# MARSLab-UMN/vi_depth_completion

Hardware: AMD Instinct MI355X
Metric: frames/sec (higher is better)
Workload: dtype f32

## Files before the change

vi_depth_completion_amd/csrc/wfused.hip:

```cpp
#include "common.h"
#include <cstdlib>

#pragma clang fp contract(off)

namespace {

typedef float f32x4 __attribute__((ext_vector_type(4)));

constexpr int TB = 16, NBW = 32, KC = 16, NPOS = 36;
constexpr int NPW = 8, NTW = 8, NTHREADS = 64 * (NPW + NTW);
constexpr int VBUF = NPOS * TB * KC;
constexpr int XSLOT = 37;
constexpr int XBUF = TB * XSLOT * KC;
constexpr int NDMA = TB * XSLOT / 16;
constexpr int MLD = 36;
constexpr size_t LDS_BYTES = (size_t)(2 * VBUF + 2 * XBUF) * sizeof(float);
static_assert(TB * XSLOT % 16 == 0, "whole DMA instructions");
static_assert((size_t)NPOS * TB * MLD * sizeof(float) <= LDS_BYTES, "the epilogue's product rows reuse the buffers");
static_assert(LDS_BYTES <= 160 * 1024, "one workgroup per CU");

struct FArgs {
    const float* x; const float* u; float* y; const float* s1; const float* b1; const float* s2; const float* b2;
    int H, W, Cin, ldx, Cout, ldy, th, tw, T, flags, nbn, gn;
    long long x_gs, w_gs, y_gs, p_gs;
    unsigned x_bytes;
};

typedef __attribute__((address_space(3))) void lds_void_t;

template <typename V> __device__ __forceinline__ void bt6_lo(const V (&d)[6], V (&t)[3]) {
    const V p = d[4] - 4.f * d[2], q = d[3] - 4.f * d[1];
    t[0] = (4.f * d[0] - 5.f * d[2]) + d[4];
    t[1] = p + q;
    t[2] = p - q;
}
template <typename V> __device__ __forceinline__ void bt6_hi(const V (&d)[6], V (&t)[3]) {
    const V r = d[4] - d[2], s = 2.f * (d[3] - d[1]);
    t[0] = r + s;
    t[1] = r - s;
    t[2] = (4.f * d[1] - 5.f * d[3]) + d[5];
}
template <typename V> __device__ __forceinline__ void bt6(const V (&d)[6], V (&t)[6]) {
    V lo[3], hi[3];
    bt6_lo(d, lo);
    bt6_hi(d, hi);
#pragma unroll
    for (int i = 0; i < 3; ++i) { t[i] = lo[i]; t[3 + i] = hi[i]; }
}
__device__ __forceinline__ void at6(const float (&m)[6], float (&o)[4]) {
    const float s12 = m[1] + m[2], d12 = m[1] - m[2], s34 = m[3] + m[4], d34 = m[3] - m[4];
    o[0] = (m[0] + s12) + s34;
    o[1] = d12 + 2.f * d34;
    o[2] = s12 + 4.f * s34;
    o[3] = (d12 + 8.f * d34) + m[5];
}

template <int N_> __device__ __forceinline__ void wait_lgkmcnt() { asm volatile("s_waitcnt lgkmcnt(%0)" ::"n"(N_) : "memory"); }
__device__ __forceinline__ f32x4 lds_read_b128(unsigned addr) {
    f32x4 v;
    asm volatile("ds_read_b128 %0, %1" : "=v"(v) : "v"(addr));
    return v;
}
template <int OFF> __device__ __forceinline__ float lds_read_b32(unsigned addr) {
    float v;
    asm volatile("ds_read_b32 %0, %1 offset:%2" : "=v"(v) : "v"(addr), "n"(OFF));
    return v;
}
template <int OFF> __device__ __forceinline__ void lds_write_b32(unsigned addr, float v) { asm volatile("ds_write_b32 %0, %1 offset:%2" ::"v"(addr), "v"(v), "n"(OFF) : "memory"); }

template <int PW, int NB, int DBG>
__device__ __forceinline__ void product_wave(const FArgs& a, float* smem, unsigned lds0, int lane, int pos0, int g, int nb, int NK) {
    const int n = lane & 15, kq = lane >> 4;
    const int n32 = a.Cout / 32, pair = NB == 2 ? nb : nb >> 1, half = NB == 2 ? 0 : nb & 1;
    const float* ub = a.u + (size_t)g * a.w_gs + ((size_t)pos0 * n32 + pair) * ((size_t)NK * 512) + half * 256 + lane * 4;
    const size_t pos_stride = (size_t)n32 * NK * 512;
    auto load_b = [&](int p, int kc, f32x4 (&dst)[NB]) {
        const float* s = ub + (size_t)p * pos_stride + (size_t)kc * 512;
        dst[0] = *reinterpret_cast<const f32x4*>(s);
        if constexpr (NB == 2) dst[1] = *reinterpret_cast<const f32x4*>(s + 256);
    };
    f32x4 acc[PW][NB];
#pragma unroll
    for (int p = 0; p < PW; ++p)
#pragma unroll
        for (int j = 0; j < NB; ++j) acc[p][j] = f32x4{0.f, 0.f, 0.f, 0.f};
    f32x4 bq[PW][NB];
#pragma unroll
    for (int p = 0; p < PW; ++p) load_b(p, 0, bq[p]);
    const unsigned a_off = (unsigned)((n * KC + ((kq ^ ((n >> 2) & 3)) * 4)) * 4);
    const unsigned a_wave = lds0 + (unsigned)(pos0 * TB * KC * 4);

    __builtin_amdgcn_s_barrier();
    __builtin_amdgcn_s_barrier();
    __builtin_amdgcn_s_barrier();
    for (int kc = 0; kc < NK; ++kc) {
        const unsigned vb = a_wave + (unsigned)((kc & 1) * VBUF * 4);
        const int kn = kc + 1 < NK ? kc + 1 : kc;
        f32x4 fa[2];
        fa[0] = lds_read_b128(vb + a_off);
#pragma unroll
        for (int p = 0; p < PW; ++p) {
            const int cur = p & 1, nxt = cur ^ 1;
            if (p + 1 < PW) {
                fa[nxt] = lds_read_b128(vb + (unsigned)((p + 1) * TB * KC * 4) + a_off);
                wait_lgkmcnt<1>();
            } else {
                wait_lgkmcnt<0>();
            }
            __builtin_amdgcn_sched_barrier(0);
#pragma unroll
            for (int ks = 0; ks < 4; ++ks)
#pragma unroll
                for (int j = 0; j < NB; ++j)
                    if constexpr (!(DBG & 1)) acc[p][j] = __builtin_amdgcn_mfma_f32_16x16x4f32(fa[cur][ks], bq[p][j][ks], acc[p][j], 0, 0, 0);
                    else if (ks == 0) acc[p][j][0] += fa[cur][0] + fa[cur][3] + bq[p][j][0] + bq[p][j][3];
            if constexpr (!(DBG & 2)) load_b(p, kn, bq[p]);
            __builtin_amdgcn_sched_barrier(0);
        }
        __builtin_amdgcn_s_barrier();
    }
    asm volatile("s_waitcnt vmcnt(0)" ::: "memory");
    float* mx = smem;
#pragma unroll
    for (int p = 0; p < PW; ++p)
#pragma unroll
        for (int j = 0; j < NB; ++j)
#pragma unroll
            for (int i = 0; i < 4; ++i) mx[((pos0 + p) * TB + 4 * kq + i) * MLD + j * 16 + n] = acc[p][j][i];
}

template <int NB, int DBG>
__global__ void __launch_bounds__(NTHREADS)
wino4_fused_kernel(const FArgs a) {
    extern __shared__ __attribute__((aligned(16))) float smem[];
    const int tid = threadIdx.x;
    const int L = blockIdx.x;
    const int tb = L / a.gn, r_ = L - tb * a.gn, g = r_ / a.nbn, nb = r_ - g * a.nbn;
    const int NK = a.Cin / KC;
    const unsigned lds0 = (unsigned)(size_t)((__attribute__((address_space(3))) float*)smem);

    if (tid < 64 * NPW) {
        const int w = __builtin_amdgcn_readfirstlane(tid >> 6);
        if (w < 4) product_wave<5, NB, DBG>(a, smem, lds0, tid & 63, 5 * w, g, nb, NK);
        else product_wave<4, NB, DBG>(a, smem, lds0, tid & 63, 20 + 4 * (w - 4), g, nb, NK);
    } else {
        const int tt = tid - 64 * NPW, lane = tid & 63;
        const int w8 = __builtin_amdgcn_readfirstlane(tt >> 6), grp = w8 >> 2;
        const int u_ = tt & 255, m = u_ >> 4, c = u_ & 15;
        const int tpf = a.th * a.tw;
        constexpr unsigned OOB = 0x80000000u;
        unsigned voff[5];
#pragma unroll
        for (int i = 0; i < 5; ++i) {
            const int j = w8 + 8 * i;
            const int slot = 16 * j + (lane >> 2), quad = lane & 3;
            const int ts = slot / XSLOT, px = slot - ts * XSLOT;
            const int t = tb * TB + ts;
            bool ok = j < NDMA && px < 36 && t < a.T;
            const int tc = ok ? t : 0;
            const int b = tc / tpf, rem = tc - b * tpf, ty = rem / a.tw, tx = rem - ty * a.tw;
            const int r = px / 6, s = px - r * 6;
            const int iy = ty * 4 - 1 + r, ix = tx * 4 - 1 + s;
            ok = ok && (unsigned)iy < (unsigned)a.H && (unsigned)ix < (unsigned)a.W;
            voff[i] = ok ? (unsigned)(((size_t)((b * a.H + iy) * a.W + ix) * a.ldx + (size_t)g * a.x_gs + quad * 4) * 4) : OOB;
        }
        const __amdgpu_buffer_rsrc_t x_rsrc = __builtin_amdgcn_make_buffer_rsrc(const_cast<float*>(a.x), 0, (int)a.x_bytes, 0x00020000);
        auto dma = [&](int cc) {
            float* dst = smem + 2 * VBUF + (cc & 1) * XBUF;
            const int soff = cc * KC * 4;
#pragma unroll
            for (int i = 0; i < 5; ++i)
                if (w8 + 8 * i < NDMA) __builtin_amdgcn_raw_ptr_buffer_load_lds(x_rsrc, (lds_void_t*)(dst + (w8 + 8 * i) * 256), 16, (int)voff[i], soff, 0, 0);
        };
        float out[36];
        const unsigned x_thr = lds0 + (unsigned)((2 * VBUF + (m * XSLOT) * KC + c) * 4);
        const unsigned v_thr = lds0 + (unsigned)((m * KC + (((c >> 2) ^ ((m >> 2) & 3)) * 4) + (c & 3)) * 4);
        auto phase_a = [&](int cc) {
            const unsigned xa = x_thr + (unsigned)((cc & 1) * XBUF * 4);
            float D[36];
#define VIDC_RD(i) D[i] = lds_read_b32<(i) * KC * 4>(xa);
            VIDC_RD(0) VIDC_RD(1) VIDC_RD(2) VIDC_RD(3) VIDC_RD(4) VIDC_RD(5) VIDC_RD(6) VIDC_RD(7) VIDC_RD(8) VIDC_RD(9) VIDC_RD(10) VIDC_RD(11)
            VIDC_RD(12) VIDC_RD(13) VIDC_RD(14) VIDC_RD(15) VIDC_RD(16) VIDC_RD(17) VIDC_RD(18) VIDC_RD(19) VIDC_RD(20) VIDC_RD(21) VIDC_RD(22) VIDC_RD(23)
            VIDC_RD(24) VIDC_RD(25) VIDC_RD(26) VIDC_RD(27) VIDC_RD(28) VIDC_RD(29) VIDC_RD(30) VIDC_RD(31) VIDC_RD(32) VIDC_RD(33) VIDC_RD(34) VIDC_RD(35)
#undef VIDC_RD
            asm volatile("s_waitcnt lgkmcnt(0)" : "+v"(D[0]), "+v"(D[1]), "+v"(D[2]), "+v"(D[3]), "+v"(D[4]), "+v"(D[5]), "+v"(D[6]), "+v"(D[7]), "+v"(D[8]), "+v"(D[9]), "+v"(D[10]), "+v"(D[11]), "+v"(D[12]), "+v"(D[13]), "+v"(D[14]), "+v"(D[15]), "+v"(D[16]), "+v"(D[17]) :: "memory");
            asm volatile("" : "+v"(D[18]), "+v"(D[19]), "+v"(D[20]), "+v"(D[21]), "+v"(D[22]), "+v"(D[23]), "+v"(D[24]), "+v"(D[25]), "+v"(D[26]), "+v"(D[27]), "+v"(D[28]), "+v"(D[29]), "+v"(D[30]), "+v"(D[31]), "+v"(D[32]), "+v"(D[33]), "+v"(D[34]), "+v"(D[35]) :: "memory");
            float tcol[6][6];
#pragma unroll
            for (int s = 0; s < 6; ++s) {
                float col[6], o6[6];
#pragma unroll
                for (int r = 0; r < 6; ++r) col[r] = D[r * 6 + s];
                bt6(col, o6);
#pragma unroll
                for (int r = 0; r < 6; ++r) tcol[r][s] = o6[r];
            }
#pragma unroll
            for (int r = 0; r < 6; ++r) {
                float o6[6];
                bt6(tcol[r], o6);
#pragma unroll
                for (int s = 0; s < 6; ++s) out[r * 6 + s] = o6[s];
            }
        };
        auto phase_b = [&](int cc) {
            const unsigned va = v_thr + (unsigned)((cc & 1) * VBUF * 4);
#define VIDC_WR(i) lds_write_b32<(i) * TB * KC * 4>(va, out[i]);
            VIDC_WR(0) VIDC_WR(1) VIDC_WR(2) VIDC_WR(3) VIDC_WR(4) VIDC_WR(5) VIDC_WR(6) VIDC_WR(7) VIDC_WR(8) VIDC_WR(9) VIDC_WR(10) VIDC_WR(11)
            VIDC_WR(12) VIDC_WR(13) VIDC_WR(14) VIDC_WR(15) VIDC_WR(16) VIDC_WR(17) VIDC_WR(18) VIDC_WR(19) VIDC_WR(20) VIDC_WR(21) VIDC_WR(22) VIDC_WR(23)
            VIDC_WR(24) VIDC_WR(25) VIDC_WR(26) VIDC_WR(27) VIDC_WR(28) VIDC_WR(29) VIDC_WR(30) VIDC_WR(31) VIDC_WR(32) VIDC_WR(33) VIDC_WR(34) VIDC_WR(35)
#undef VIDC_WR
        };
        auto fence_barrier = [&]() {
            if constexpr (DBG & 16) asm volatile("s_waitcnt lgkmcnt(0)" ::: "memory");
            else asm volatile("s_waitcnt vmcnt(0) lgkmcnt(0)" ::: "memory");
            __builtin_amdgcn_s_barrier();
        };
        dma(0);
        if (NK > 1) dma(1);
        fence_barrier();
        if (grp == 0) phase_a(0);
        else if (NK > 1) phase_a(1);
        fence_barrier();
        if (NK > 2) dma(2);
        if (grp == 0) phase_b(0);
        fence_barrier();
        for (int it = 0; it < NK; ++it) {
            if (!(DBG & 4)) {
                if (it + 3 < NK) dma(it + 3);
                if ((it & 1) == grp) {
                    if (it + 2 < NK) phase_a(it + 2);
                } else {
                    if (it + 1 < NK) phase_b(it + 1);
                }
            }
            fence_barrier();
        }
    }
    __syncthreads();
    if (tid < TB * 16 * NB) {
        const int m = tid / (16 * NB), c = tid - m * (16 * NB);
        const int t = tb * TB + m;
        if (t >= a.T || (DBG & 8)) return;
        const int tpf = a.th * a.tw;
        const int b = t / tpf, rem = t - b * tpf, ty = rem / a.tw, tx = rem - ty * a.tw;
        const float* mx = smem + m * MLD + c;
        float tc[4][6];
#pragma unroll
        for (int s = 0; s < 6; ++s) {
            float col[6], o4[4];
#pragma unroll
            for (int r = 0; r < 6; ++r) col[r] = mx[(r * 6 + s) * TB * MLD];
            at6(col, o4);
#pragma unroll
            for (int r = 0; r < 4; ++r) tc[r][s] = o4[r];
        }
        const int ch = nb * 16 * NB + c;
        const float s1 = a.s1[(size_t)g * a.p_gs + ch], b1 = a.b1[(size_t)g * a.p_gs + ch];
        const bool aff2 = a.flags & VIDC_AFFINE2;
        const float s2 = aff2 ? a.s2[(size_t)g * a.p_gs + ch] : 0.f, b2 = aff2 ? a.b2[(size_t)g * a.p_gs + ch] : 0.f;
        const float lo1 = (a.flags & VIDC_RELU1) ? 0.f : -INFINITY, lo2 = (a.flags & VIDC_RELU2) ? 0.f : -INFINITY;
        float* yb = a.y + (size_t)g * a.y_gs + ch;
#pragma unroll
        for (int r = 0; r < 4; ++r) {
            float o4[4];
            at6(tc[r], o4);
            const int oy = ty * 4 + r;
            if (oy >= a.H) continue;
#pragma unroll
            for (int s = 0; s < 4; ++s) {
                const int ox = tx * 4 + s;
                if (ox >= a.W) continue;
                float o = fmaxf(o4[s] * s1 + b1, lo1);
                if (aff2) o = fmaxf(o * s2 + b2, lo2);
                yb[((size_t)(b * a.H + oy) * a.W + ox) * a.ldy] = o;
            }
        }
    }
}

__global__ void __launch_bounds__(256)
wino4_pack_kernel(const float* __restrict__ u, float* __restrict__ o, int Cout, int Cin, long long total4) {
    const long long i = (long long)blockIdx.x * blockDim.x + threadIdx.x;
    if (i >= total4) return;
    const int NK = Cin / KC, nbn = Cout / NBW;
    const int lane = (int)(i & 63), nblk = (int)((i >> 6) & 1);
    long long r = i >> 7;
    const int kc = (int)(r % NK); r /= NK;
    const int nb = (int)(r % nbn);
    const int pos = (int)(r / nbn);
    const int n = lane & 15, kq = lane >> 4;
    const float4 v = *reinterpret_cast<const float4*>(u + ((size_t)pos * Cout + nb * NBW + nblk * 16 + n) * Cin + kc * KC + kq * 4);
    *reinterpret_cast<float4*>(o + i * 4) = v;
}

template <int NB, int DBG>
int launch_nb(const FArgs& a, long long wgs, hipStream_t st) {
    static bool attr_set[64] = {};
    int dev = 0;
    VIDC_HIP(hipGetDevice(&dev));
    if (dev < 0 || dev >= 64 || !attr_set[dev]) {
        VIDC_HIP(hipFuncSetAttribute(reinterpret_cast<const void*>(&wino4_fused_kernel<NB, DBG>), hipFuncAttributeMaxDynamicSharedMemorySize, (int)LDS_BYTES));
        if (dev >= 0 && dev < 64) attr_set[dev] = true;
    }
    hipLaunchKernelGGL((wino4_fused_kernel<NB, DBG>), dim3((unsigned)wgs), dim3(NTHREADS), LDS_BYTES, st, a);
    VIDC_CHECK_LAUNCH("wino4_fused_kernel");
    return VIDC_OK;
}

template <int DBG>
int launch_dbg(const FArgs& a, long long wgs, hipStream_t st) { return a.nbn * 32 == a.Cout ? launch_nb<2, DBG>(a, wgs, st) : launch_nb<1, DBG>(a, wgs, st); }

}

namespace vidc {

int launch_wino4_fused(const vidc_conv_desc& d, hipStream_t st) {
    VIDC_REQUIRE(d.precision == VIDC_PREC_FP32, VIDC_ERR_SHAPE, "conv (fused Winograd): fp32 arithmetic only");
    VIDC_REQUIRE(d.KH == 3 && d.KW == 3 && d.stride == 1 && d.pad == 1 && d.dilation <= 1, VIDC_ERR_SHAPE, "conv (fused Winograd): 3x3 / stride 1 / pad 1 / dense only");
    VIDC_REQUIRE(d.Cin % KC == 0 && d.Cout % NBW == 0 && d.ldx % 4 == 0, VIDC_ERR_SHAPE, "conv (fused Winograd): Cin %% 16 == 0, Cout %% 32 == 0, ldx %% 4 == 0");
    VIDC_REQUIRE(!(d.flags & ~(VIDC_RELU1 | VIDC_AFFINE2 | VIDC_RELU2)), VIDC_ERR_SHAPE, "conv (fused Winograd): flags 0x%x not supported (affine / ReLU / second affine / ReLU only)", d.flags);
    VIDC_REQUIRE(d.w_gs == (long long)NPOS * d.Cout * d.Cin || d.groups == 1, VIDC_ERR_SHAPE, "conv (fused Winograd): w = U of vidc_winograd_weight_pack_fused, w_gs = 36 * Cout * Cin");
    VIDC_REQUIRE((reinterpret_cast<uintptr_t>(d.x) & 15) == 0 && (reinterpret_cast<uintptr_t>(d.w) & 15) == 0 && d.x_gs % 4 == 0, VIDC_ERR_SHAPE, "conv (fused Winograd): x and U 16-byte aligned");
    FArgs a;
    a.x = d.x; a.u = d.w; a.y = d.y; a.s1 = d.scale1; a.b1 = d.shift1; a.s2 = d.scale2; a.b2 = d.shift2;
    a.H = d.H; a.W = d.W; a.Cin = d.Cin; a.ldx = d.ldx; a.Cout = d.Cout; a.ldy = d.ldy;
    a.th = (d.H + 3) / 4; a.tw = (d.W + 3) / 4;
    a.T = d.B * a.th * a.tw;
    static const int force_nb = [] { const char* e = getenv("VIDC_WFUSED_NB"); return e ? atoi(e) : 0; }();
    const long long wgs32 = (long long)((d.B * a.th * a.tw + TB - 1) / TB) * d.groups * (d.Cout / NBW);
    const int nbk = force_nb == 1 || force_nb == 2 ? force_nb : (wgs32 * 2 <= 256 ? 1 : 2);
    a.flags = d.flags; a.nbn = d.Cout / (16 * nbk); a.gn = d.groups * a.nbn;
    a.x_gs = d.x_gs; a.w_gs = d.w_gs; a.y_gs = d.y_gs; a.p_gs = d.p_gs;
    VIDC_REQUIRE((long long)d.B * d.H * d.W * d.ldx * 4 < (1ll << 30), VIDC_ERR_SHAPE, "conv (fused Winograd): the input must stay below 1 GiB");
    a.x_bytes = (unsigned)((long long)d.B * d.H * d.W * d.ldx * 4);
    const long long wgs = (long long)((a.T + TB - 1) / TB) * a.gn;
    VIDC_REQUIRE(wgs < (1ll << 31), VIDC_ERR_SHAPE, "conv (fused Winograd): grid too large");
#ifdef VIDC_WFUSED_ATTRIB
    static const int dbg = [] { const char* e = getenv("VIDC_WFUSED_DBG"); return e ? atoi(e) : 0; }();
    switch (dbg) {
        case 1: return launch_dbg<1>(a, wgs, st);
        case 2: return launch_dbg<2>(a, wgs, st);
        case 4: return launch_dbg<4>(a, wgs, st);
        case 8: return launch_dbg<8>(a, wgs, st);
        case 3: return launch_dbg<3>(a, wgs, st);
        case 6: return launch_dbg<6>(a, wgs, st);
        case 7: return launch_dbg<7>(a, wgs, st);
        case 15: return launch_dbg<15>(a, wgs, st);
        case 16: return launch_dbg<16>(a, wgs, st);
        default: break;
    }
#endif
    return launch_dbg<0>(a, wgs, st);
}

}

extern "C" int vidc_winograd_weight_pack_fused(const float* u, float* u_packed, int Cout, int Cin, vidc_stream_t stream) {
    VIDC_REQUIRE(u && u_packed && u != u_packed, VIDC_ERR_NULL, "vidc_winograd_weight_pack_fused: null pointer (or in place)");
    VIDC_REQUIRE(Cout > 0 && Cin > 0 && Cout % NBW == 0 && Cin % KC == 0, VIDC_ERR_SHAPE, "vidc_winograd_weight_pack_fused: Cout must be a multiple of 32, Cin of 16");
    const long long total4 = (long long)NPOS * Cout * Cin / 4;
    hipLaunchKernelGGL(wino4_pack_kernel, dim3((unsigned)((total4 + 255) / 256)), dim3(256), 0, vidc::as_stream(stream), u, u_packed, Cout, Cin, total4);
    VIDC_CHECK_LAUNCH("wino4_pack_kernel");
    return VIDC_OK;
}
```

Baseline: 632.0.

## Make fused Winograd conv persistent for Cin=64 with cross-item prefetch

For Cin==64 layers the fused Winograd kernel now launches a grid sized to the CU count, rounded to a multiple of groups*nbn, and loops over tile items. Each workgroup prefetches the next item's first input chunks and weight slices while the current item's K loop finishes, so the pipeline does not drain and refill between tiles. This aims to cut workgroup launch and prologue cost. The epilogue is moved into a shared fold_store, and the product rows are stored in a compact XOR-swizzled layout that fits in the V buffers. In exchange there are extra block-wide syncs per item and possible load imbalance on the last round of items.

Result: faster. 639.5, median of 6 (+1.2%).

```diff
diff --git a/vi_depth_completion_amd/csrc/wfused.hip b/vi_depth_completion_amd/csrc/wfused.hip
--- a/vi_depth_completion_amd/csrc/wfused.hip
+++ b/vi_depth_completion_amd/csrc/wfused.hip
@@ -18,10 +18,12 @@
 static_assert(TB * XSLOT % 16 == 0, "whole DMA instructions");
 static_assert((size_t)NPOS * TB * MLD * sizeof(float) <= LDS_BYTES, "the epilogue's product rows reuse the buffers");
 static_assert(LDS_BYTES <= 160 * 1024, "one workgroup per CU");
+static_assert(NPOS * TB * 32 <= 2 * VBUF, "a persistent workgroup's product rows fit in the two V buffers");
 
 struct FArgs {
     const float* x; const float* u; float* y; const float* s1; const float* b1; const float* s2; const float* b2;
     int H, W, Cin, ldx, Cout, ldy, th, tw, T, flags, nbn, gn;
+    int items;
     long long x_gs, w_gs, y_gs, p_gs;
     unsigned x_bytes;
 };
@@ -68,9 +70,17 @@
 }
 template <int OFF> __device__ __forceinline__ void lds_write_b32(unsigned addr, float v) { asm volatile("ds_write_b32 %0, %1 offset:%2" ::"v"(addr), "v"(v), "n"(OFF) : "memory"); }
 
-template <int PW, int NB, int DBG>
-__device__ __forceinline__ void product_wave(const FArgs& a, float* smem, unsigned lds0, int lane, int pos0, int g, int nb, int NK) {
+template <bool PERSIST> __device__ __forceinline__ int prow(int pos, int m, int col) {
+    if constexpr (PERSIST) return (pos * TB + m) * 32 + (col ^ (((m >> 2) & 1) << 4));
+    else return (pos * TB + m) * MLD + col;
+}
+
+template <int NB, int DBG, bool PERSIST> __device__ void fold_store(const FArgs& a, const float* smem, int tid, int tb, int g, int nb);
+template <int PW, int NB, int DBG, bool PERSIST>
+__device__ __forceinline__ void product_wave(const FArgs& a, float* smem, unsigned lds0, int tid, int pos0, int NK) {
+    const int lane = tid & 63;
     const int n = lane & 15, kq = lane >> 4;
+    const int item0 = blockIdx.x, r0 = item0 % a.gn, g = r0 / a.nbn, nb = r0 - g * a.nbn;
     const int n32 = a.Cout / 32, pair = NB == 2 ? nb : nb >> 1, half = NB == 2 ? 0 : nb & 1;
     const float* ub = a.u + (size_t)g * a.w_gs + ((size_t)pos0 * n32 + pair) * ((size_t)NK * 512) + half * 256 + lane * 4;
     const size_t pos_stride = (size_t)n32 * NK * 512;
@@ -79,77 +89,123 @@
         dst[0] = *reinterpret_cast<const f32x4*>(s);
         if constexpr (NB == 2) dst[1] = *reinterpret_cast<const f32x4*>(s + 256);
     };
-    f32x4 acc[PW][NB];
-#pragma unroll
-    for (int p = 0; p < PW; ++p)
-#pragma unroll
-        for (int j = 0; j < NB; ++j) acc[p][j] = f32x4{0.f, 0.f, 0.f, 0.f};
     f32x4 bq[PW][NB];
 #pragma unroll
     for (int p = 0; p < PW; ++p) load_b(p, 0, bq[p]);
     const unsigned a_off = (unsigned)((n * KC + ((kq ^ ((n >> 2) & 3)) * 4)) * 4);
     const unsigned a_wave = lds0 + (unsigned)(pos0 * TB * KC * 4);
 
-    __builtin_amdgcn_s_barrier();
-    __builtin_amdgcn_s_barrier();
-    __builtin_amdgcn_s_barrier();
-    for (int kc = 0; kc < NK; ++kc) {
-        const unsigned vb = a_wave + (unsigned)((kc & 1) * VBUF * 4);
-        const int kn = kc + 1 < NK ? kc + 1 : kc;
-        f32x4 fa[2];
-        fa[0] = lds_read_b128(vb + a_off);
-#pragma unroll
-        for (int p = 0; p < PW; ++p) {
-            const int cur = p & 1, nxt = cur ^ 1;
-            if (p + 1 < PW) {
-                fa[nxt] = lds_read_b128(vb + (unsigned)((p + 1) * TB * KC * 4) + a_off);
-                wait_lgkmcnt<1>();
-            } else {
-                wait_lgkmcnt<0>();
+    for (int item = item0; item < a.items; item += gridDim.x) {
+        const bool more = PERSIST && item + (int)gridDim.x < a.items;
+        f32x4 acc[PW][NB];
+#pragma unroll
+        for (int p = 0; p < PW; ++p)
+#pragma unroll
+            for (int j = 0; j < NB; ++j) acc[p][j] = f32x4{0.f, 0.f, 0.f, 0.f};
+        __builtin_amdgcn_s_barrier();
+        __builtin_amdgcn_s_barrier();
+        __builtin_amdgcn_s_barrier();
+        for (int kc = 0; kc < NK; ++kc) {
+            const unsigned vb = a_wave + (unsigned)((kc & 1) * VBUF * 4);
+            const int kn = kc + 1 < NK ? kc + 1 : (more ? 0 : kc);
+            f32x4 fa[2];
+            fa[0] = lds_read_b128(vb + a_off);
+#pragma unroll
+            for (int p = 0; p < PW; ++p) {
+                const int cur = p & 1, nxt = cur ^ 1;
+                if (p + 1 < PW) {
+                    fa[nxt] = lds_read_b128(vb + (unsigned)((p + 1) * TB * KC * 4) + a_off);
+                    wait_lgkmcnt<1>();
+                } else {
+                    wait_lgkmcnt<0>();
+                }
+                __builtin_amdgcn_sched_barrier(0);
+#pragma unroll
+                for (int ks = 0; ks < 4; ++ks)
+#pragma unroll
+                    for (int j = 0; j < NB; ++j)
+                        if constexpr (!(DBG & 1)) acc[p][j] = __builtin_amdgcn_mfma_f32_16x16x4f32(fa[cur][ks], bq[p][j][ks], acc[p][j], 0, 0, 0);
+                        else if (ks == 0) acc[p][j][0] += fa[cur][0] + fa[cur][3] + bq[p][j][0] + bq[p][j][3];
+                if constexpr (!(DBG & 2)) load_b(p, kn, bq[p]);
+                __builtin_amdgcn_sched_barrier(0);
             }
-            __builtin_amdgcn_sched_barrier(0);
-#pragma unroll
-            for (int ks = 0; ks < 4; ++ks)
-#pragma unroll
-                for (int j = 0; j < NB; ++j)
-                    if constexpr (!(DBG & 1)) acc[p][j] = __builtin_amdgcn_mfma_f32_16x16x4f32(fa[cur][ks], bq[p][j][ks], acc[p][j], 0, 0, 0);
-                    else if (ks == 0) acc[p][j][0] += fa[cur][0] + fa[cur][3] + bq[p][j][0] + bq[p][j][3];
-            if constexpr (!(DBG & 2)) load_b(p, kn, bq[p]);
-            __builtin_amdgcn_sched_barrier(0);
-        }
-        __builtin_amdgcn_s_barrier();
-    }
-    asm volatile("s_waitcnt vmcnt(0)" ::: "memory");
-    float* mx = smem;
-#pragma unroll
-    for (int p = 0; p < PW; ++p)
-#pragma unroll
-        for (int j = 0; j < NB; ++j)
-#pragma unroll
-            for (int i = 0; i < 4; ++i) mx[((pos0 + p) * TB + 4 * kq + i) * MLD + j * 16 + n] = acc[p][j][i];
-}
-
-template <int NB, int DBG>
+            __builtin_amdgcn_s_barrier();
+        }
+        asm volatile("s_waitcnt vmcnt(0)" ::: "memory");
+#pragma unroll
+        for (int p = 0; p < PW; ++p)
+#pragma unroll
+            for (int j = 0; j < NB; ++j)
+#pragma unroll
+                for (int i = 0; i < 4; ++i) smem[prow<PERSIST>(pos0 + p, 4 * kq + i, j * 16 + n)] = acc[p][j][i];
+        __syncthreads();
+        fold_store<NB, DBG, PERSIST>(a, smem, tid, item / a.gn, g, nb);
+        if constexpr (PERSIST) __syncthreads();
+    }
+}
+
+template <int NB, int DBG, bool PERSIST>
+__device__ void fold_store(const FArgs& a, const float* smem, int tid, int tb, int g, int nb) {
+    if (tid >= TB * 16 * NB) return;
+    const int m = tid / (16 * NB), c = tid - m * (16 * NB);
+    const int t = tb * TB + m;
+    if (t >= a.T || (DBG & 8)) return;
+    const int tpf = a.th * a.tw;
+    const int b = t / tpf, rem = t - b * tpf, ty = rem / a.tw, tx = rem - ty * a.tw;
+    float tc[4][6];
+#pragma unroll
+    for (int s = 0; s < 6; ++s) {
+        float col[6], o4[4];
+#pragma unroll
+        for (int r = 0; r < 6; ++r) col[r] = smem[prow<PERSIST>(r * 6 + s, m, c)];
+        at6(col, o4);
+#pragma unroll
+        for (int r = 0; r < 4; ++r) tc[r][s] = o4[r];
+    }
+    const int ch = nb * 16 * NB + c;
+    const float s1 = a.s1[(size_t)g * a.p_gs + ch], b1 = a.b1[(size_t)g * a.p_gs + ch];
+    const bool aff2 = a.flags & VIDC_AFFINE2;
+    const float s2 = aff2 ? a.s2[(size_t)g * a.p_gs + ch] : 0.f, b2 = aff2 ? a.b2[(size_t)g * a.p_gs + ch] : 0.f;
+    const float lo1 = (a.flags & VIDC_RELU1) ? 0.f : -INFINITY, lo2 = (a.flags & VIDC_RELU2) ? 0.f : -INFINITY;
+    float* yb = a.y + (size_t)g * a.y_gs + ch;
+#pragma unroll
+    for (int r = 0; r < 4; ++r) {
+        float o4[4];
+        at6(tc[r], o4);
+        const int oy = ty * 4 + r;
+        if (oy >= a.H) continue;
+#pragma unroll
+        for (int s = 0; s < 4; ++s) {
+            const int ox = tx * 4 + s;
+            if (ox >= a.W) continue;
+            float o = fmaxf(o4[s] * s1 + b1, lo1);
+            if (aff2) o = fmaxf(o * s2 + b2, lo2);
+            yb[((size_t)(b * a.H + oy) * a.W + ox) * a.ldy] = o;
+        }
+    }
+}
+
+template <int NB, int DBG, bool PERSIST>
 __global__ void __launch_bounds__(NTHREADS)
 wino4_fused_kernel(const FArgs a) {
     extern __shared__ __attribute__((aligned(16))) float smem[];
     const int tid = threadIdx.x;
-    const int L = blockIdx.x;
-    const int tb = L / a.gn, r_ = L - tb * a.gn, g = r_ / a.nbn, nb = r_ - g * a.nbn;
     const int NK = a.Cin / KC;
     const unsigned lds0 = (unsigned)(size_t)((__attribute__((address_space(3))) float*)smem);
 
     if (tid < 64 * NPW) {
         const int w = __builtin_amdgcn_readfirstlane(tid >> 6);
-        if (w < 4) product_wave<5, NB, DBG>(a, smem, lds0, tid & 63, 5 * w, g, nb, NK);
-        else product_wave<4, NB, DBG>(a, smem, lds0, tid & 63, 20 + 4 * (w - 4), g, nb, NK);
-    } else {
-        const int tt = tid - 64 * NPW, lane = tid & 63;
-        const int w8 = __builtin_amdgcn_readfirstlane(tt >> 6), grp = w8 >> 2;
-        const int u_ = tt & 255, m = u_ >> 4, c = u_ & 15;
-        const int tpf = a.th * a.tw;
-        constexpr unsigned OOB = 0x80000000u;
-        unsigned voff[5];
+        if (w < 4) product_wave<5, NB, DBG, PERSIST>(a, smem, lds0, tid, 5 * w, NK);
+        else product_wave<4, NB, DBG, PERSIST>(a, smem, lds0, tid, 20 + 4 * (w - 4), NK);
+        return;
+    }
+    const int tt = tid - 64 * NPW, lane = tid & 63;
+    const int w8 = __builtin_amdgcn_readfirstlane(tt >> 6), grp = w8 >> 2;
+    const int u_ = tt & 255, m = u_ >> 4, c = u_ & 15;
+    const int tpf = a.th * a.tw;
+    const int g = (blockIdx.x % a.gn) / a.nbn;
+    constexpr unsigned OOB = 0x80000000u;
+    auto offsets = [&](int tb, unsigned (&voff)[5]) {
 #pragma unroll
         for (int i = 0; i < 5; ++i) {
             const int j = w8 + 8 * i;
@@ -164,70 +220,83 @@
             ok = ok && (unsigned)iy < (unsigned)a.H && (unsigned)ix < (unsigned)a.W;
             voff[i] = ok ? (unsigned)(((size_t)((b * a.H + iy) * a.W + ix) * a.ldx + (size_t)g * a.x_gs + quad * 4) * 4) : OOB;
         }
-        const __amdgpu_buffer_rsrc_t x_rsrc = __builtin_amdgcn_make_buffer_rsrc(const_cast<float*>(a.x), 0, (int)a.x_bytes, 0x00020000);
-        auto dma = [&](int cc) {
-            float* dst = smem + 2 * VBUF + (cc & 1) * XBUF;
-            const int soff = cc * KC * 4;
-#pragma unroll
-            for (int i = 0; i < 5; ++i)
-                if (w8 + 8 * i < NDMA) __builtin_amdgcn_raw_ptr_buffer_load_lds(x_rsrc, (lds_void_t*)(dst + (w8 + 8 * i) * 256), 16, (int)voff[i], soff, 0, 0);
-        };
-        float out[36];
-        const unsigned x_thr = lds0 + (unsigned)((2 * VBUF + (m * XSLOT) * KC + c) * 4);
-        const unsigned v_thr = lds0 + (unsigned)((m * KC + (((c >> 2) ^ ((m >> 2) & 3)) * 4) + (c & 3)) * 4);
-        auto phase_a = [&](int cc) {
-            const unsigned xa = x_thr + (unsigned)((cc & 1) * XBUF * 4);
-            float D[36];
+    };
+    const __amdgpu_buffer_rsrc_t x_rsrc = __builtin_amdgcn_make_buffer_rsrc(const_cast<float*>(a.x), 0, (int)a.x_bytes, 0x00020000);
+    auto dma = [&](const unsigned (&voff)[5], int cc) {
+        float* dst = smem + 2 * VBUF + (cc & 1) * XBUF;
+        const int soff = cc * KC * 4;
+#pragma unroll
+        for (int i = 0; i < 5; ++i)
+            if (w8 + 8 * i < NDMA) __builtin_amdgcn_raw_ptr_buffer_load_lds(x_rsrc, (lds_void_t*)(dst + (w8 + 8 * i) * 256), 16, (int)voff[i], soff, 0, 0);
+    };
+    float out[36];
+    const unsigned x_thr = lds0 + (unsigned)((2 * VBUF + (m * XSLOT) * KC + c) * 4);
+    const unsigned v_thr = lds0 + (unsigned)((m * KC + (((c >> 2) ^ ((m >> 2) & 3)) * 4) + (c & 3)) * 4);
+    auto phase_a = [&](int cc) {
+        const unsigned xa = x_thr + (unsigned)((cc & 1) * XBUF * 4);
+        float D[36];
 #define VIDC_RD(i) D[i] = lds_read_b32<(i) * KC * 4>(xa);
-            VIDC_RD(0) VIDC_RD(1) VIDC_RD(2) VIDC_RD(3) VIDC_RD(4) VIDC_RD(5) VIDC_RD(6) VIDC_RD(7) VIDC_RD(8) VIDC_RD(9) VIDC_RD(10) VIDC_RD(11)
-            VIDC_RD(12) VIDC_RD(13) VIDC_RD(14) VIDC_RD(15) VIDC_RD(16) VIDC_RD(17) VIDC_RD(18) VIDC_RD(19) VIDC_RD(20) VIDC_RD(21) VIDC_RD(22) VIDC_RD(23)
-            VIDC_RD(24) VIDC_RD(25) VIDC_RD(26) VIDC_RD(27) VIDC_RD(28) VIDC_RD(29) VIDC_RD(30) VIDC_RD(31) VIDC_RD(32) VIDC_RD(33) VIDC_RD(34) VIDC_RD(35)
+        VIDC_RD(0) VIDC_RD(1) VIDC_RD(2) VIDC_RD(3) VIDC_RD(4) VIDC_RD(5) VIDC_RD(6) VIDC_RD(7) VIDC_RD(8) VIDC_RD(9) VIDC_RD(10) VIDC_RD(11)
+        VIDC_RD(12) VIDC_RD(13) VIDC_RD(14) VIDC_RD(15) VIDC_RD(16) VIDC_RD(17) VIDC_RD(18) VIDC_RD(19) VIDC_RD(20) VIDC_RD(21) VIDC_RD(22) VIDC_RD(23)
+        VIDC_RD(24) VIDC_RD(25) VIDC_RD(26) VIDC_RD(27) VIDC_RD(28) VIDC_RD(29) VIDC_RD(30) VIDC_RD(31) VIDC_RD(32) VIDC_RD(33) VIDC_RD(34) VIDC_RD(35)
 #undef VIDC_RD
-            asm volatile("s_waitcnt lgkmcnt(0)" : "+v"(D[0]), "+v"(D[1]), "+v"(D[2]), "+v"(D[3]), "+v"(D[4]), "+v"(D[5]), "+v"(D[6]), "+v"(D[7]), "+v"(D[8]), "+v"(D[9]), "+v"(D[10]), "+v"(D[11]), "+v"(D[12]), "+v"(D[13]), "+v"(D[14]), "+v"(D[15]), "+v"(D[16]), "+v"(D[17]) :: "memory");
-            asm volatile("" : "+v"(D[18]), "+v"(D[19]), "+v"(D[20]), "+v"(D[21]), "+v"(D[22]), "+v"(D[23]), "+v"(D[24]), "+v"(D[25]), "+v"(D[26]), "+v"(D[27]), "+v"(D[28]), "+v"(D[29]), "+v"(D[30]), "+v"(D[31]), "+v"(D[32]), "+v"(D[33]), "+v"(D[34]), "+v"(D[35]) :: "memory");
-            float tcol[6][6];
-#pragma unroll
-            for (int s = 0; s < 6; ++s) {
-                float col[6], o6[6];
-#pragma unroll
-                for (int r = 0; r < 6; ++r) col[r] = D[r * 6 + s];
-                bt6(col, o6);
-#pragma unroll
-                for (int r = 0; r < 6; ++r) tcol[r][s] = o6[r];
-            }
-#pragma unroll
-            for (int r = 0; r < 6; ++r) {
-                float o6[6];
-                bt6(tcol[r], o6);
-#pragma unroll
-                for (int s = 0; s < 6; ++s) out[r * 6 + s] = o6[s];
-            }
-        };
-        auto phase_b = [&](int cc) {
-            const unsigned va = v_thr + (unsigned)((cc & 1) * VBUF * 4);
+        asm volatile("s_waitcnt lgkmcnt(0)" : "+v"(D[0]), "+v"(D[1]), "+v"(D[2]), "+v"(D[3]), "+v"(D[4]), "+v"(D[5]), "+v"(D[6]), "+v"(D[7]), "+v"(D[8]), "+v"(D[9]), "+v"(D[10]), "+v"(D[11]), "+v"(D[12]), "+v"(D[13]), "+v"(D[14]), "+v"(D[15]), "+v"(D[16]), "+v"(D[17]) :: "memory");
+        asm volatile("" : "+v"(D[18]), "+v"(D[19]), "+v"(D[20]), "+v"(D[21]), "+v"(D[22]), "+v"(D[23]), "+v"(D[24]), "+v"(D[25]), "+v"(D[26]), "+v"(D[27]), "+v"(D[28]), "+v"(D[29]), "+v"(D[30]), "+v"(D[31]), "+v"(D[32]), "+v"(D[33]), "+v"(D[34]), "+v"(D[35]) :: "memory");
+        float tcol[6][6];
+#pragma unroll
+        for (int s = 0; s < 6; ++s) {
+            float col[6], o6[6];
+#pragma unroll
+            for (int r = 0; r < 6; ++r) col[r] = D[r * 6 + s];
+            bt6(col, o6);
+#pragma unroll
+            for (int r = 0; r < 6; ++r) tcol[r][s] = o6[r];
+        }
+#pragma unroll
+        for (int r = 0; r < 6; ++r) {
+            float o6[6];
+            bt6(tcol[r], o6);
+#pragma unroll
+            for (int s = 0; s < 6; ++s) out[r * 6 + s] = o6[s];
+        }
+    };
+    auto phase_b = [&](int cc) {
+        const unsigned va = v_thr + (unsigned)((cc & 1) * VBUF * 4);
 #define VIDC_WR(i) lds_write_b32<(i) * TB * KC * 4>(va, out[i]);
-            VIDC_WR(0) VIDC_WR(1) VIDC_WR(2) VIDC_WR(3) VIDC_WR(4) VIDC_WR(5) VIDC_WR(6) VIDC_WR(7) VIDC_WR(8) VIDC_WR(9) VIDC_WR(10) VIDC_WR(11)
-            VIDC_WR(12) VIDC_WR(13) VIDC_WR(14) VIDC_WR(15) VIDC_WR(16) VIDC_WR(17) VIDC_WR(18) VIDC_WR(19) VIDC_WR(20) VIDC_WR(21) VIDC_WR(22) VIDC_WR(23)
-            VIDC_WR(24) VIDC_WR(25) VIDC_WR(26) VIDC_WR(27) VIDC_WR(28) VIDC_WR(29) VIDC_WR(30) VIDC_WR(31) VIDC_WR(32) VIDC_WR(33) VIDC_WR(34) VIDC_WR(35)
+        VIDC_WR(0) VIDC_WR(1) VIDC_WR(2) VIDC_WR(3) VIDC_WR(4) VIDC_WR(5) VIDC_WR(6) VIDC_WR(7) VIDC_WR(8) VIDC_WR(9) VIDC_WR(10) VIDC_WR(11)
+        VIDC_WR(12) VIDC_WR(13) VIDC_WR(14) VIDC_WR(15) VIDC_WR(16) VIDC_WR(17) VIDC_WR(18) VIDC_WR(19) VIDC_WR(20) VIDC_WR(21) VIDC_WR(22) VIDC_WR(23)
+        VIDC_WR(24) VIDC_WR(25) VIDC_WR(26) VIDC_WR(27) VIDC_WR(28) VIDC_WR(29) VIDC_WR(30) VIDC_WR(31) VIDC_WR(32) VIDC_WR(33) VIDC_WR(34) VIDC_WR(35)
 #undef VIDC_WR
-        };
-        auto fence_barrier = [&]() {
-            if constexpr (DBG & 16) asm volatile("s_waitcnt lgkmcnt(0)" ::: "memory");
-            else asm volatile("s_waitcnt vmcnt(0) lgkmcnt(0)" ::: "memory");
-            __builtin_amdgcn_s_barrier();
-        };
-        dma(0);
-        if (NK > 1) dma(1);
+    };
+    auto fence_barrier = [&]() {
+        if constexpr (DBG & 16) asm volatile("s_waitcnt lgkmcnt(0)" ::: "memory");
+        else asm volatile("s_waitcnt vmcnt(0) lgkmcnt(0)" ::: "memory");
+        __builtin_amdgcn_s_barrier();
+    };
+    unsigned voff[5], vnext[5];
+    offsets(blockIdx.x / a.gn, voff);
+    for (int item = blockIdx.x; item < a.items; item += gridDim.x) {
+        const bool first = item == (int)blockIdx.x, more = PERSIST && item + (int)gridDim.x < a.items;
+        if (!first) {
+#pragma unroll
+            for (int i = 0; i < 5; ++i) voff[i] = vnext[i];
+        }
+        if (more) offsets((item + (int)gridDim.x) / a.gn, vnext);
+        if (first) {
+            dma(voff, 0);
+            if (NK > 1) dma(voff, 1);
+        }
         fence_barrier();
         if (grp == 0) phase_a(0);
         else if (NK > 1) phase_a(1);
         fence_barrier();
-        if (NK > 2) dma(2);
+        if (NK > 2) dma(voff, 2);
         if (grp == 0) phase_b(0);
         fence_barrier();
         for (int it = 0; it < NK; ++it) {
             if (!(DBG & 4)) {
-                if (it + 3 < NK) dma(it + 3);
+                if (it + 3 < NK) dma(voff, it + 3);
+                else if (more && it + 3 - NK < 2) dma(vnext, it + 3 - NK);
                 if ((it & 1) == grp) {
                     if (it + 2 < NK) phase_a(it + 2);
                 } else {
@@ -236,46 +305,8 @@
             }
             fence_barrier();
         }
-    }
-    __syncthreads();
-    if (tid < TB * 16 * NB) {
-        const int m = tid / (16 * NB), c = tid - m * (16 * NB);
-        const int t = tb * TB + m;
-        if (t >= a.T || (DBG & 8)) return;
-        const int tpf = a.th * a.tw;
-        const int b = t / tpf, rem = t - b * tpf, ty = rem / a.tw, tx = rem - ty * a.tw;
-        const float* mx = smem + m * MLD + c;
-        float tc[4][6];
-#pragma unroll
-        for (int s = 0; s < 6; ++s) {
-            float col[6], o4[4];
-#pragma unroll
-            for (int r = 0; r < 6; ++r) col[r] = mx[(r * 6 + s) * TB * MLD];
-            at6(col, o4);
-#pragma unroll
-            for (int r = 0; r < 4; ++r) tc[r][s] = o4[r];
-        }
-        const int ch = nb * 16 * NB + c;
-        const float s1 = a.s1[(size_t)g * a.p_gs + ch], b1 = a.b1[(size_t)g * a.p_gs + ch];
-        const bool aff2 = a.flags & VIDC_AFFINE2;
-        const float s2 = aff2 ? a.s2[(size_t)g * a.p_gs + ch] : 0.f, b2 = aff2 ? a.b2[(size_t)g * a.p_gs + ch] : 0.f;
-        const float lo1 = (a.flags & VIDC_RELU1) ? 0.f : -INFINITY, lo2 = (a.flags & VIDC_RELU2) ? 0.f : -INFINITY;
-        float* yb = a.y + (size_t)g * a.y_gs + ch;
-#pragma unroll
-        for (int r = 0; r < 4; ++r) {
-            float o4[4];
-            at6(tc[r], o4);
-            const int oy = ty * 4 + r;
-            if (oy >= a.H) continue;
-#pragma unroll
-            for (int s = 0; s < 4; ++s) {
-                const int ox = tx * 4 + s;
-                if (ox >= a.W) continue;
-                float o = fmaxf(o4[s] * s1 + b1, lo1);
-                if (aff2) o = fmaxf(o * s2 + b2, lo2);
-                yb[((size_t)(b * a.H + oy) * a.W + ox) * a.ldy] = o;
-            }
-        }
+        __syncthreads();
+        if constexpr (PERSIST) __syncthreads();
     }
 }
 
@@ -294,22 +325,25 @@
     *reinterpret_cast<float4*>(o + i * 4) = v;
 }
 
-template <int NB, int DBG>
+template <int NB, int DBG, bool PERSIST>
 int launch_nb(const FArgs& a, long long wgs, hipStream_t st) {
     static bool attr_set[64] = {};
     int dev = 0;
     VIDC_HIP(hipGetDevice(&dev));
     if (dev < 0 || dev >= 64 || !attr_set[dev]) {
-        VIDC_HIP(hipFuncSetAttribute(reinterpret_cast<const void*>(&wino4_fused_kernel<NB, DBG>), hipFuncAttributeMaxDynamicSharedMemorySize, (int)LDS_BYTES));
+        VIDC_HIP(hipFuncSetAttribute(reinterpret_cast<const void*>(&wino4_fused_kernel<NB, DBG, PERSIST>), hipFuncAttributeMaxDynamicSharedMemorySize, (int)LDS_BYTES));
         if (dev >= 0 && dev < 64) attr_set[dev] = true;
     }
-    hipLaunchKernelGGL((wino4_fused_kernel<NB, DBG>), dim3((unsigned)wgs), dim3(NTHREADS), LDS_BYTES, st, a);
+    hipLaunchKernelGGL((wino4_fused_kernel<NB, DBG, PERSIST>), dim3((unsigned)wgs), dim3(NTHREADS), LDS_BYTES, st, a);
     VIDC_CHECK_LAUNCH("wino4_fused_kernel");
     return VIDC_OK;
 }
 
 template <int DBG>
-int launch_dbg(const FArgs& a, long long wgs, hipStream_t st) { return a.nbn * 32 == a.Cout ? launch_nb<2, DBG>(a, wgs, st) : launch_nb<1, DBG>(a, wgs, st); }
+int launch_dbg(const FArgs& a, long long wgs, bool persist, hipStream_t st) {
+    if (persist) return a.nbn * 32 == a.Cout ? launch_nb<2, DBG, true>(a, wgs, st) : launch_nb<1, DBG, true>(a, wgs, st);
+    return a.nbn * 32 == a.Cout ? launch_nb<2, DBG, false>(a, wgs, st) : launch_nb<1, DBG, false>(a, wgs, st);
+}
 
 }
 
@@ -334,24 +368,44 @@
     a.x_gs = d.x_gs; a.w_gs = d.w_gs; a.y_gs = d.y_gs; a.p_gs = d.p_gs;
     VIDC_REQUIRE((long long)d.B * d.H * d.W * d.ldx * 4 < (1ll << 30), VIDC_ERR_SHAPE, "conv (fused Winograd): the input must stay below 1 GiB");
     a.x_bytes = (unsigned)((long long)d.B * d.H * d.W * d.ldx * 4);
-    const long long wgs = (long long)((a.T + TB - 1) / TB) * a.gn;
-    VIDC_REQUIRE(wgs < (1ll << 31), VIDC_ERR_SHAPE, "conv (fused Winograd): grid too large");
+    const long long items = (long long)((a.T + TB - 1) / TB) * a.gn;
+    VIDC_REQUIRE(items < (1ll << 31), VIDC_ERR_SHAPE, "conv (fused Winograd): grid too large");
+    a.items = (int)items;
+    long long wgs = items;
+    bool persist = false;
+    if (d.Cin == 64) {
+        static int n_cu[64] = {};
+        int dev = 0;
+        VIDC_HIP(hipGetDevice(&dev));
+        int cus = dev >= 0 && dev < 64 ? n_cu[dev] : 0;
+        if (cus == 0) {
+            VIDC_HIP(hipDeviceGetAttribute(&cus, hipDeviceAttributeMultiprocessorCount, dev));
+            if (dev >= 0 && dev < 64) n_cu[dev] = cus;
+        }
+        long long q = a.gn;
+        while (q % 8) q += a.gn;
+        const long long grid = (cus / q) * q;
+        if (grid > 0 && items > grid) {
+            wgs = grid;
+            persist = true;
+        }
+    }
 #ifdef VIDC_WFUSED_ATTRIB
     static const int dbg = [] { const char* e = getenv("VIDC_WFUSED_DBG"); return e ? atoi(e) : 0; }();
     switch (dbg) {
-        case 1: return launch_dbg<1>(a, wgs, st);
-        case 2: return launch_dbg<2>(a, wgs, st);
-        case 4: return launch_dbg<4>(a, wgs, st);
-        case 8: return launch_dbg<8>(a, wgs, st);
-        case 3: return launch_dbg<3>(a, wgs, st);
-        case 6: return launch_dbg<6>(a, wgs, st);
-        case 7: return launch_dbg<7>(a, wgs, st);
-        case 15: return launch_dbg<15>(a, wgs, st);
-        case 16: return launch_dbg<16>(a, wgs, st);
+        case 1: return launch_dbg<1>(a, wgs, persist, st);
+        case 2: return launch_dbg<2>(a, wgs, persist, st);
+        case 4: return launch_dbg<4>(a, wgs, persist, st);
+        case 8: return launch_dbg<8>(a, wgs, persist, st);
+        case 3: return launch_dbg<3>(a, wgs, persist, st);
+        case 6: return launch_dbg<6>(a, wgs, persist, st);
+        case 7: return launch_dbg<7>(a, wgs, persist, st);
+        case 15: return launch_dbg<15>(a, wgs, persist, st);
+        case 16: return launch_dbg<16>(a, wgs, persist, st);
         default: break;
     }
 #endif
-    return launch_dbg<0>(a, wgs, st);
+    return launch_dbg<0>(a, wgs, persist, st);
 }
 
 }
```
